# poloclub/3d-gaussian-splat-attack

Hardware: AMD Instinct MI355X
Metric: fwd+bwd views/sec @1080p, 1M Gaussians (higher is better)
Workload: dtype f32; 1 GPU; S-nyc-1M: 1000000 Gaussians (SH degree 3), 1920x1080, one view per step per GPU, render() fwd + bwd to all attribute grads, object channels off; P=1000000, width=1920, height=1080, loop=independent views, views_per_rank=1, views_per_launch_chain=1, cameras=the 8 ring cameras in turn, streams=4, parallelism=views sharded 1/GPU, dp1, independent views pipelined over 4 HIP streams per GPU

## Files before the change

3d-gaussian-splat-attack_amd/csrc/gsr_api.hip:

```cpp
#include <hip/hip_runtime.h>
#include <hip/hip_ext.h>

#include <algorithm>
#include <atomic>
#include <cfloat>
#include <cmath>
#include <cstdarg>
#include <cstdio>
#include <cstdlib>
#include <cstring>
#include <chrono>
#include <mutex>
#include <thread>
#include <new>
#include <vector>

#include "../../include/gsraster.h"
#include "gsr_kernels.hip.h"
#include "gsr_sort.hip.h"
#include "gsr_knn.hip.h"
#include "gsr_pgd.hip.h"
#include "gsr_groups.hip.h"
#include "gsr_hull.h"
#include "gsr_image.hip.h"
// ... 227 lines not shown
    const CapKey& q = g_caps[i].k;
    if (q.dev == k.dev && q.P == k.P && q.H == k.H && q.W == k.W) {
      if (erase) { g_caps[i] = g_caps.back(); g_caps.pop_back(); }
      else g_caps[i].n = n;
      return;
    }
  }
  if (!erase) {
    if (g_caps.size() >= 256) g_caps.clear();
    g_caps.push_back(CapEntry{k, n});
  }
}

struct SideStream { int dev; hipStream_t main, side; hipEvent_t fork, join; };
std::mutex g_side_mu;
std::vector<SideStream> g_sides;

bool side_stream_for(int dev, hipStream_t main, SideStream& out) {
  std::lock_guard<std::mutex> lk(g_side_mu);
  for (const SideStream& s : g_sides)
    if (s.dev == dev && s.main == main) { out = s; return true; }
  SideStream s{dev, main, nullptr, nullptr, nullptr};
  int least = 0, greatest = 0;
  if (hipDeviceGetStreamPriorityRange(&least, &greatest) != hipSuccess) { (void)hipGetLastError(); least = 0; }
  if (hipStreamCreateWithPriority(&s.side, hipStreamNonBlocking, least) != hipSuccess ||
      hipEventCreateWithFlags(&s.fork, hipEventDisableTiming) != hipSuccess ||
      hipEventCreateWithFlags(&s.join, hipEventDisableTiming) != hipSuccess) {
    (void)hipGetLastError();
    return false;
  }
  g_sides.push_back(s);
  out = s;
  return true;
}

struct PendingSlot { CountSlot slot; CapKey key; };
std::mutex g_pending_mu;
std::vector<PendingSlot> g_pending;

void pending_harvest() {
  std::lock_guard<std::mutex> lk(g_pending_mu);
  for (size_t i = 0; i < g_pending.size();) {
    PendingSlot& ps = g_pending[i];
    if (slot_landed(ps.slot)) {
      const unsigned long long n = (unsigned long long)ps.slot.host[HS_N64] | ((unsigned long long)ps.slot.host[HS_N64 + 1] << 32);
      cap_store(ps.key, n, ps.slot.host[HS_OVF] != 0u);
      slot_put(ps.slot);
      g_pending[i] = g_pending.back();
      g_pending.pop_back();
    } else {
      ++i;
    }
  }
}

struct ProfSpan { int stage; hipEvent_t a, b; };
std::mutex g_prof_mu;
uint32_t g_prof = 0;
std::vector<ProfSpan> g_spans;
std::vector<hipEvent_t> g_free_events;
float g_ms[GSR_STAGE_COUNT] = {0};
int64_t g_calls[GSR_STAGE_COUNT] = {0};

hipEvent_t get_event_locked() {
  if (!g_free_events.empty()) { hipEvent_t e = g_free_events.back(); g_free_events.pop_back(); return e; }
  hipEvent_t e;
// ... 429 lines not shown
  }
};

int FwdRun::allocate() {
  c = new (std::nothrow) GsrCtx();
  if (!c) return set_err(GSR_ERR_NOMEM, "gsr_forward: host allocation failed");
  c->dev = dev; c->st = *f.s; c->P = p.P; c->K = p.K; c->gridx = p.gridx; c->gridy = p.gridy; c->ntiles = p.ntiles;
  c->B = p.B; c->Ppad = p.Ppad; c->Pv = p.Pv; c->tpv = p.tpv;
  if (p.B > 1) c->views.assign(f.s, f.s + p.B);
  c->means3D = f.means3D; c->shs = f.shs; c->sh_objs = p.sh_objs; c->colors = f.colors_precomp; c->opac = f.opacities;
  c->scales = f.scales; c->rots = f.rotations; c->cov3d = f.cov3D_precomp;
  c->raw = f.raw; c->sh_dc = f.sh_dc;
  c->fwd_only = f.fwd_only; c->objects_out = f.out_objects != nullptr && p.sh_objs != nullptr;
  c->aux = f.out_depth != nullptr || f.out_alpha != nullptr; c->aux_depth_out = f.out_depth; c->aux_alpha_out = f.out_alpha;
  if (f.segb) { c->has_b = true; c->b = *f.segb; }
  c->lanegroup = p.lanegroup;
  c->depth_passes = p.depth_passes; c->group_sums = p.group_sums; c->scan_items = scan_items_for((uint32_t)p.Pv);
  Slab ksize, ssize;
  keep_regions(ksize, p, c);
  scratch_regions(ssize, p, w);
  c->keep_bytes = ksize.block_bytes();
  c->keep_blk = pool_alloc(dev, c->keep_bytes, st);
  scratch_blk = pool_alloc(dev, ssize.block_bytes(), st);
  if (!c->keep_blk || !scratch_blk)
    return set_err(GSR_ERR_NOMEM, "gsr_forward: workspace allocation failed (P=%d, %dx%d)", p.P, p.W, p.H);
  Slab ks(c->keep_blk, c->keep_bytes), ss(scratch_blk, ssize.block_bytes());
  keep_regions(ks, p, c);
  scratch_regions(ss, p, w);
  if (!ks.ok || !ss.ok) return set_err(GSR_ERR_STATE, "gsr_forward: a workspace region ends beyond its block");
  return GSR_OK;
}

int FwdRun::fork_color() {
  static const int side_env = [] { const char* e = getenv("GSR_SIDE_STREAM"); return e ? atoi(e) : 1; }();
  hipStream_t cs = st;
  if (side_env != 0 && !(f.s->flags & GSR_FLAG_NO_SIDE_STREAM) && side_stream_for(dev, st, side)) {
    HIP_TRY("side stream", hipEventRecord(side.fork, st));
    HIP_TRY("side stream", hipStreamWaitEvent(side.side, side.fork, 0));
    cs = side.side;
    side_used = true;
  }
  constexpr unsigned COLOR_BLOCKS = 512;
  const dim3 gridC(side_used ? std::min<unsigned>(p.nkc, COLOR_BLOCKS) : p.nkc), blkCol(PREF_BLOCK);
  if (p.B > 1) hipLaunchKernelGGL(k_pre_color_batch, gridC, blkCol, 0, cs, color_batch_args(c, w.tcnt));
  else hipLaunchKernelGGL(f.raw ? k_pre_color<true> : k_pre_color<false>, gridC, blkCol, 0, cs, color_args(c, w.tcnt));
  if (side_used) HIP_TRY("side stream", hipEventRecord(side.join, side.side));
  return GSR_OK;
}

int FwdRun::preprocess() {
  const int ntiles = p.ntiles;
  StageTimer t(GSR_STAGE_PREPROCESS, st);
  PreBlockOut bo;
  bo.bout = w.bout;
  bo.ranges = p.P >= p.tpv ? c->ranges : nullptr;
  bo.ntiles = p.tpv;
  if (!bo.ranges) {
    HIP_TRY("ranges", hipMemset2DAsync(c->ranges, sizeof(uint2), 0xFF, sizeof(uint32_t), ntiles, st));
    HIP_TRY("ranges", hipMemset2DAsync(reinterpret_cast<char*>(c->ranges) + sizeof(uint32_t), sizeof(uint2), 0, sizeof(uint32_t), ntiles, st));
  }
  if (p.B > 1) launch_pack_views(c, st);
  if (c->lanegroup) {
    PreArgs pa = color_args(c, w.tcnt);
    pa.Pfill = p.B > 1 ? p.Ppad : p.P; pa.vpack = p.B > 1 ? c->vpack : nullptr; pa.bpv = (int)p.nk1v;
    pa.scales = f.scales; pa.rots = f.rotations; pa.cov3d = f.cov3D_precomp; pa.opac = f.opacities;
    pa.colors = f.colors_precomp; pa.radii = f.radii; pa.dkey = w.dkey; pa.tcnt8 = w.tcnt8; pa.abc = c->abc;
    pa.scales_b = f.segb ? f.segb->scaling : nullptr; pa.rots_b = f.segb ? f.segb->rotation : nullptr;
    pa.opac_b = f.segb ? f.segb->opacity : nullptr;
    pa.cull = p.cull; pa.bo = bo;
// ... 447 lines not shown
  if (c->P > 0) {
    StageTimer t(GSR_STAGE_PREPROCESS, st);
    const bool skip_D = (flags & GSR_RERENDER_COLOR_GRADS_ONLY) != 0u;
    c->D_stale = c->D != nullptr && skip_D;
    const bool first_only = c->has_b && (flags & GSR_RERENDER_FIRST_SEGMENT_ONLY);
    const dim3 blkC(PREF_BLOCK);
    if (c->B > 1) {
      launch_pack_views(c, st);
      PreColorBatchArgs ca = color_batch_args(c, nullptr);
      if (first_only) ca.P = ca.Pa;
      if (skip_D) ca.D = nullptr;
      hipLaunchKernelGGL(k_pre_color_batch, dim3((unsigned)((ca.P + PREF_BLOCK - 1) / PREF_BLOCK)), blkC, 0, st, ca);
    } else {
      PreArgs pa = color_args(c, nullptr);
      if (first_only) pa.P = pa.Pa;
      if (skip_D) pa.D = nullptr;
      hipLaunchKernelGGL(c->raw ? k_pre_color<true> : k_pre_color<false>, dim3((unsigned)((pa.P + PREF_BLOCK - 1) / PREF_BLOCK)), blkC, 0, st, pa);
    }
    hipError_t e = hipGetLastError();
    if (e != hipSuccess)
      return set_err(GSR_ERR_DEVICE, "rerender colours%s: launch failed: %s", c->B > 1 ? " (batch)" : "", hipGetErrorString(e));
  }
  StageTimer t(GSR_STAGE_RENDER_FWD, st);
  return launch_render_fwd(c, out_color, out_objects, st);
}

}

static bool batch_k9_fused() {
  static const int env = [] { const char* e = getenv("GSR_BATCH_K9"); return e ? atoi(e) : 1; }();
  return env != 0;
}

struct GradOut {
  float *means3D = nullptr, *means2D = nullptr, *shs = nullptr, *sh_dc = nullptr, *sh_objs = nullptr,
        *colors_precomp = nullptr, *opacities = nullptr, *scales = nullptr, *rotations = nullptr, *cov3D = nullptr;
};

struct BwdCall {
  const float *grad_color = nullptr, *grad_objects = nullptr;
  GradOut d;
  bool accumulate = false;
  int nchunks = 1;
  gsr_chunk_fn chunk_done = nullptr;
  void* chunk_user = nullptr;
  int64_t view_stride = 0;
  void* stream = nullptr;
};

static int check_ctx_kind(const char* fn, const GsrCtx* c, bool want_raw) {
  if (!c || c->raw == want_raw) return GSR_OK;
  if (!want_raw) return set_err(GSR_ERR_STATE, "%s: context came from gsr_forward_raw; use gsr_backward_raw", fn);
  return set_err(GSR_ERR_STATE, "%s: context came from gsr_forward; use gsr_backward", fn);
}

struct BwdRun {
  GsrCtx* c;
  const BwdCall& b;
  hipStream_t st;
  double* ss_out = nullptr;
  const float *aux_gd = nullptr, *aux_ga = nullptr;
  bool aux = false;
  bool obj = false;
  bool geom = false;
  int nchunks = 1;
  bool batch_fused = false;
  bool segs_on = false;
  int bwd_npx = 4;
  uint32_t nsub = 1;
  uint32_t tag_lo = 0, tag_hi = 0;
  float4 *part = nullptr, *part_obj = nullptr;
  int finish(int code) { pool_free(c->dev, part); pool_free(c->dev, part_obj); return code; }

  int check_aux_grads() const;
  int check_pre_bwd();
  int take_partial_rows();
  int render_bwd();
  int pre_bwd();
  PreBwdArgs shared_args() const;
  void launch_batch(const PreBwdArgs& sh, int gb, int ge) const;
  void launch_views(PreBwdArgs pa, int gb, int ge) const;
  void launch_view(PreBwdArgs pa, int v, int gb, int ge) const;
};

int BwdRun::check_aux_grads() const {
  if (b.view_stride != 0)
    return set_err(GSR_ERR_INVALID, "gsr_ctx_set_aux_grads: the per-view batch backward (gsr_backward_raw_batch_views / _obj_views) "
                   "does not take depth / alpha gradients");
  if (b.nchunks > 1)
    return set_err(GSR_ERR_INVALID, "gsr_ctx_set_aux_grads: gsr_backward_raw_chunked with more than one range does not take "
                   "depth / alpha gradients");
  if (b.grad_objects != nullptr)
    return set_err(GSR_ERR_INVALID, "gsr_ctx_set_aux_grads: depth / alpha gradients and grad_objects in one backward are not supported");
  if (!geom)
    return set_err(GSR_ERR_INVALID, "gsr_ctx_set_aux_grads: depth / alpha gradients reach geometry and opacity only, and this "
                   "backward asks for no such gradient");
  if (!c->lanegroup)
    return set_err(GSR_ERR_INVALID, "gsr_ctx_set_aux_grads: a gsr_forward context with K != 16 SH coefficients does not take "
                   "depth / alpha gradients");
  if (c->st.flags & GSR_FLAG_NEEDLE_DOUBLE)
    return set_err(GSR_ERR_INVALID, "gsr_ctx_set_aux_grads: not available under GSR_FLAG_NEEDLE_DOUBLE");
  return GSR_OK;
}

int BwdRun::check_pre_bwd() {
  const float* const dsh = c->shs ? b.d.shs : nullptr;
  if (c->raw && ((dsh == nullptr) != (b.d.sh_dc == nullptr)))
    return set_err(GSR_ERR_INVALID, "gsr_backward_raw: dfeatures_dc and dfeatures_rest must both be given");
  if (c->lanegroup && c->shs && geom && !c->D)
    return set_err(GSR_ERR_STATE, "gsr_backward: the forward of this context was run without its backward state");
  if (c->lanegroup && c->shs && geom && c->D_stale)
    return set_err(GSR_ERR_STATE, "gsr_backward: geometry gradients asked of a context whose last gsr_ctx_rerender was "
                   "told GSR_RERENDER_COLOR_GRADS_ONLY");
  nchunks = std::max(1, std::min(b.nchunks, (c->P + 63) / 64));
  batch_fused = c->B > 1 && c->raw && c->lanegroup && batch_k9_fused() && b.view_stride == 0;
  if (ss_out && (!(c->lanegroup && c->raw) || b.accumulate || nchunks != 1 || (c->B > 1 && !batch_fused)))
    return set_err(GSR_ERR_INVALID, "gsr_ctx_request_sumsq: served by an overwriting gsr_backward_raw* over one range only");
  return GSR_OK;
}

int BwdRun::take_partial_rows() {
  const uint32_t N = c->nbound;
  segs_on = c->bnd != nullptr && !obj && aux_gd == nullptr;
  bwd_npx = flag_bwd_npx(c->st.flags) ? flag_bwd_npx(c->st.flags) : ((c->tpv < 4096 && !segs_on) ? 2 : 4);
  nsub = (uint32_t)(PXL / bwd_npx);
  if (N > 0) {
    part = static_cast<float4*>(pool_alloc(c->dev, sizeof(float4) * PART_F4 * (size_t)N * nsub, st));
    if (obj) part_obj = static_cast<float4*>(pool_alloc(c->dev, sizeof(float4) * 4 * (size_t)N * nsub, st));
    if (!part || (obj && !part_obj))
      return set_err(GSR_ERR_NOMEM, "gsr_backward: partial-gradient buffer (N=%u) allocation failed", N);
  }
  static std::atomic<uint64_t> tag_counter{0x243F6A8885A308D3ull};
  uint64_t z = tag_counter.fetch_add(0x9E3779B97F4A7C15ull) + 0x9E3779B97F4A7C15ull;
  z = (z ^ (z >> 30)) * 0xBF58476D1CE4E5B9ull; z = (z ^ (z >> 27)) * 0x94D049BB133111EBull; z ^= z >> 31;
  tag_lo = (uint32_t)z; tag_hi = (uint32_t)(z >> 32);
  return GSR_OK;
}

int BwdRun::render_bwd() {
  StageTimer t(GSR_STAGE_RENDER_BWD, st, true);
  RenderBwdArgs ra;
  ra.tag_lo = tag_lo; ra.tag_hi = tag_hi;
  ra.ranges = c->ranges; ra.pair_rank = c->pair_rank; ra.offg = c->offg; ra.R0 = c->G0; ra.R1 = c->G1; ra.R2 = c->G2;
  ra.sh_objs = c->sh_objs; ra.bg = c->st.bg; ra.W = c->st.image_width; ra.H = c->st.image_height;
  ra.map_mode = flag_tile_map(c->st.flags);
  ra.sched = c->sched;
  ra.wave_clock = g_wave_clock.load();
  ra.gridx = c->gridx; ra.ntiles = c->ntiles; ra.final_T = c->final_T; ra.n_contrib = c->n_contrib;
  ra.grad_color = b.grad_color; ra.grad_objects = obj ? b.grad_objects : nullptr; ra.part = part; ra.part_obj = part_obj;
  ra.grad_depth = aux_gd; ra.grad_alpha = aux_ga;
  ra.bnd = segs_on ? c->bnd : nullptr; ra.segoff = c->segoff; ra.rec_item = c->rec_item; ra.nrec = c->dv + DV_NREC;
  ra.seg_shift = c->seg_shift; ra.extra_blocks = segs_on ? c->rec_cap * nsub : 0u;
  ra.tpv = c->tpv; ra.vpack = c->vpack; ra.Ppad = c->Ppad;
  const dim3 gridT(ra.extra_blocks + (unsigned)render_grid(c->ntiles * (int)nsub)), blk(64);
  const Kern<RenderBwdArgs> k7 = pick_render_bwd(obj, bwd_npx, geom, aux);
  if (t.on) hipExtLaunchKernelGGL(k7, gridT, blk, 0, st, t.a, t.b, 0, ra);
  else hipLaunchKernelGGL(k7, gridT, blk, 0, st, ra);
  LAUNCH_CHECK("render backward");
  return GSR_OK;
}

PreBwdArgs BwdRun::shared_args() const {
  const GradOut& g = b.d;
  PreBwdArgs pa;
  pa.P = c->P; pa.g0 = 0; pa.K = c->K; pa.va = view_args(c->st);
  pa.offg = c->offg; pa.G0 = c->G0; pa.G1 = c->G1; pa.G2 = c->G2;
  pa.part = part; pa.part_obj = obj ? part_obj : nullptr;
  pa.tag_lo = tag_lo; pa.tag_hi = tag_hi; pa.nsub = nsub;
  pa.means = c->means3D; pa.scales = c->scales; pa.rots = c->rots; pa.cov3d = c->cov3d; pa.sh = c->shs;
  pa.sh_dc = c->sh_dc; pa.D = c->D; pa.abc = c->abc;
  pa.needle_double = (c->st.flags & GSR_FLAG_NEEDLE_DOUBLE) != 0u ? 1 : 0;
  pa.dmeans3D = g.means3D; pa.dmeans2D = g.means2D; pa.dsh = c->shs ? g.shs : nullptr; pa.dsh_dc = g.sh_dc;
  pa.dsh_objs = c->B > 1 ? nullptr : g.sh_objs; pa.dcolors = c->colors ? g.colors_precomp : nullptr; pa.dopac = g.opacities;
  pa.dscales = c->cov3d ? nullptr : g.scales; pa.drots = c->cov3d ? nullptr : g.rotations;
  pa.dcov3d = c->cov3d ? g.cov3D : nullptr;
  pa.accumulate = b.accumulate ? 1 : 0;
  pa.vpack = nullptr; pa.Ppad = 0; pa.Pscene = c->P; pa.vstride = 0;
  pa.sumsq = nullptr;
  return pa;
}

void BwdRun::launch_batch(const PreBwdArgs& sh, int gb, int ge) const {
  const GradOut& d = b.d;
  PreBwdBatchArgs ba;
  ba.P = ge; ba.g0 = gb; ba.B = c->B; ba.Ppad = c->Ppad; ba.Pscene = c->P; ba.vpack = c->vpack;
  ba.H = c->st.image_height; ba.W = c->st.image_width; ba.deg = c->st.sh_degree; ba.mod = c->st.scale_modifier;
  ba.offg = c->offg; ba.G0 = c->G0; ba.G1 = c->G1; ba.G2 = c->G2; ba.part = part;
  ba.tag_lo = tag_lo; ba.tag_hi = tag_hi; ba.nsub = nsub;
  ba.means = c->means3D; ba.scales = c->scales; ba.rots = c->rots; ba.D = c->D;
  ba.dmeans3D = d.means3D; ba.dmeans2D = d.means2D; ba.dsh = d.shs; ba.dsh_dc = d.sh_dc; ba.dopac = d.opacities;
  ba.dscales = d.scales; ba.drots = d.rotations; ba.sumsq = sh.sumsq;
  const dim3 gridB((unsigned)((ge - gb + 63) / 64)), blkB(64 * BATCH_K9_WAVES);
  const size_t lds = sizeof(float) * 3 * 64 * (size_t)c->B;
  hipLaunchKernelGGL(pick_pre_bwd_batch(geom, b.accumulate, aux), gridB, blkB, lds, st, ba);
}

void BwdRun::launch_views(PreBwdArgs pa, int gb, int ge) const {
  pa.vpack = c->vpack; pa.Ppad = c->Ppad; pa.Pscene = c->P; pa.vstride = (long long)b.view_stride;
  pa.accumulate = 0; pa.abc = nullptr;
  pa.g0 = gb; pa.P = ge;
  const dim3 gridV((unsigned)((ge - gb + PRE_BLOCK - 1) / PRE_BLOCK), (unsigned)c->B);
  hipLaunchKernelGGL(pick_pre_bwd(true, geom, false, false, false), gridV, dim3(PRE_BLOCK), 0, st, pa);
}

void BwdRun::launch_view(PreBwdArgs pa, int v, int gb, int ge) const {
  const GradOut& d = b.d;
  const bool acc_v = b.view_stride == 0 && (b.accumulate || v > 0);
  if (c->B > 1) {
    const size_t o = (size_t)v * (size_t)c->Ppad;
    pa.va = view_args(c->views[v]);
    pa.offg = c->offg + o; pa.G0 = c->G0 + REC * o; pa.G1 = c->G1 + REC * o; pa.G2 = c->G2 + REC * o;
    pa.D = c->D ? c->D + 9 * o : nullptr; pa.abc = c->abc ? c->abc + o : nullptr;
    pa.dmeans2D = d.means2D ? d.means2D + 3 * (size_t)v * (size_t)c->P : nullptr;
    pa.accumulate = acc_v ? 1 : 0;
  }
  pa.g0 = gb; pa.P = ge;
  const dim3 gridK9((unsigned)((ge - gb + PRE_BLOCK - 1) / PRE_BLOCK));
  if (c->lanegroup) {
    const bool ndl = pa.needle_double != 0 && pa.abc != nullptr;
    hipLaunchKernelGGL(pick_pre_bwd(c->raw, geom, acc_v, ndl, aux), gridK9, dim3(PRE_BLOCK), 0, st, pa);
  } else {
    if (geom && pa.needle_double) hipLaunchKernelGGL((k_preprocess_bwd<true, true>), gridK9, dim3(PRE_BLOCK), 0, st, pa);
    else if (geom) hipLaunchKernelGGL((k_preprocess_bwd<true>), gridK9, dim3(PRE_BLOCK), 0, st, pa);
    else hipLaunchKernelGGL((k_preprocess_bwd<false>), gridK9, dim3(PRE_BLOCK), 0, st, pa);
  }
}

int BwdRun::pre_bwd() {
  const int P = c->P, dev = c->dev;
  StageTimer t(GSR_STAGE_PREPROCESS_BWD, st);
  PreBwdArgs pa = shared_args();
  if (c->B > 1 && b.d.sh_objs) {
// ... 24 lines not shown
  if (ss_out) {
    hipLaunchKernelGGL(k_sumsq_reduce, dim3(6), dim3(256), 0, st, pa.sumsq, ss_blocks * PRE_WAVES, ss_out);
    pool_free(dev, ss_blk);
  }
  LAUNCH_CHECK("preprocess backward");
  return GSR_OK;
}

static int backward_impl(GsrCtx* c, const BwdCall& b) {
  if (!c) return set_err(GSR_ERR_STATE, "gsr_backward: null context");
  BwdRun r{c, b, static_cast<hipStream_t>(b.stream)};
  r.ss_out = c->sumsq_out;
  c->sumsq_out = nullptr;
  r.aux_gd = c->aux_gd; r.aux_ga = c->aux_ga;
  c->aux_gd = nullptr; c->aux_ga = nullptr;
  r.aux = r.aux_gd != nullptr || r.aux_ga != nullptr;
  if (!b.grad_color) return set_err(GSR_ERR_INVALID, "gsr_backward: grad_color is null");
  if (c->fwd_only)
    return set_err(GSR_ERR_STATE, "gsr_backward: the context was kept by gsr_forward_raw2_keep (re-render only, no backward state)");
  if (c->P == 0) return GSR_OK;
  const GradOut& d = b.d;
  r.obj = b.grad_objects != nullptr && c->sh_objs != nullptr;
  r.geom = d.means3D || d.means2D || d.opacities || d.scales || d.rotations || d.cov3D;
  if (r.aux) { if (const int rc = r.check_aux_grads()) return rc; }
  if (ctx_resolve_count(c) != GSR_OK) return set_err(GSR_ERR_DEVICE, "gsr_backward: reading the forward's pair count failed");
  if (c->overflow)
    return set_err(GSR_ERR_OVERFLOW, "gsr_backward: the forward emitted %llu (tile, Gaussian) pairs, more than the capacity "
                   "%u guessed from earlier views (GSR_FLAG_ASYNC_COUNT); its image was filled with NaN -- render again",
                   c->n64, c->nbound);
  if (const int rc = r.check_pre_bwd()) return rc;
  pool_retag(c->dev, c->keep_blk, r.st); pool_retag(c->dev, c->rank_blk, r.st); pool_retag(c->dev, c->seg_blk, r.st);
  int rc;
  if ((rc = r.take_partial_rows()) != GSR_OK) return r.finish(rc);
  if (c->nbound > 0 && (rc = r.render_bwd()) != GSR_OK) return r.finish(rc);
  if ((rc = r.pre_bwd()) != GSR_OK) return r.finish(rc);
  return r.finish(GSR_OK);
}

static inline size_t det_round(size_t v) { return (v + 255) & ~(size_t)255; }

struct Carve {
  char* base;
  size_t off = 0;
  explicit Carve(void* ws = nullptr) : base(static_cast<char*>(ws)) {}
  template <class T>
  T* take(size_t count) {
    T* p = base ? reinterpret_cast<T*>(base + off) : nullptr;
    off += det_round(count * sizeof(T));
    return p;
  }
};

static int check_workspace(const char* fn, const void* ws, int64_t ws_bytes, size_t need, unsigned align, const char* sizer) {
  if (ws_bytes < (int64_t)need)
    return set_err(GSR_ERR_INVALID, "%s: workspace of %lld bytes, %zu needed (%s)", fn, (long long)ws_bytes, need, sizer);
  if (((uintptr_t)ws & (uintptr_t)(align - 1)) != 0)
    return set_err(GSR_ERR_INVALID, "%s: the workspace must be %u-byte aligned", fn, align);
  return GSR_OK;
}

template <class... P>
static int check_aligned4(const char* fn, const P*... p) {
  if (((... | (uintptr_t)p) & 3) != 0) return set_err(GSR_ERR_INVALID, "%s: every tensor must be 4-byte aligned", fn);
  return GSR_OK;
}

// ... 1623 lines not shown
```

3d-gaussian-splat-attack_amd/csrc/gsr_kernels.hip.h:

```cpp
#pragma once
#include <hip/hip_runtime.h>
#include <stdint.h>

#include "gsr_math.h"
#include "gsr_sort.hip.h"

namespace gsr {

struct ViewArgs {
  const float* vm;
  const float* pm;
  const float* cam;
  int H, W;
  float tanfovx, tanfovy, mod;
  int deg;
};

__device__ __forceinline__ void load_view(View& v, const ViewArgs& a) {
  make_view(v, a.vm, a.pm, a.cam, a.H, a.W, a.tanfovx, a.tanfovy, a.mod, a.deg);
}

constexpr int MAX_BATCH = 16;
constexpr int BATCH_PAD = 16384;
struct ViewDev {
// ... 1193 lines not shown
  ViewArgs va;
  const uint32_t* offg;
  const float4* G0;
  const float4* G1;
  const float4* G2;
  const float4* part;
  const float4* part_obj;
  uint32_t tag_lo, tag_hi;
  uint32_t nsub;
  const float* means;
  const float* scales;
  const float* rots;
  const float* cov3d;
  const float* sh;
  const float* sh_dc;
  const float* D;
  const double* abc;
  float* dmeans3D;
  float* dmeans2D;
  float* dsh;
  float* dsh_dc;
  float* dsh_objs;
  float* dcolors;
  float* dopac;
  float* dscales;
  float* drots;
  float* dcov3d;
  int accumulate;
  int needle_double;
  float* sumsq;
  const ViewDev* vpack;
  int Ppad, Pscene;
  long long vstride;
};
enum { SUMSQ_XYZ = 0, SUMSQ_DC = 1, SUMSQ_REST = 2, SUMSQ_OPACITY = 3, SUMSQ_SCALING = 4, SUMSQ_ROTATION = 5, SUMSQ_W = 8 };

__global__ void __launch_bounds__(256) k_sumsq_reduce(const float* __restrict__ part, int nblocks, double* __restrict__ out) {
  __shared__ double wsum[4];
  const int k = blockIdx.x;
  double acc = 0.0;
  for (int i = threadIdx.x; i < nblocks; i += 256) acc += (double)part[(size_t)i * SUMSQ_W + k];
#pragma unroll
  for (int s = 32; s > 0; s >>= 1) acc += __shfl_xor(acc, s, 64);
  if ((threadIdx.x & 63) == 0) wsum[threadIdx.x >> 6] = acc;
  __syncthreads();
  if (threadIdx.x == 0) out[k] = (wsum[0] + wsum[1]) + (wsum[2] + wsum[3]);
}

template <bool GEOM, bool NDL = false>
__global__ void __launch_bounds__(PRE_BLOCK) k_preprocess_bwd(PreBwdArgs a) {
  const int g = a.g0 + blockIdx.x * PRE_BLOCK + threadIdx.x;
  const int K = a.K;
  if (g >= a.P) return;
  const uint32_t o0 = a.offg[g] * a.nsub, o1 = a.offg[g + 1] * a.nsub;
  if (o1 == o0) {
    if (a.dmeans3D) { a.dmeans3D[3 * g] = 0.f; a.dmeans3D[3 * g + 1] = 0.f; a.dmeans3D[3 * g + 2] = 0.f; }
    if (a.dmeans2D) { a.dmeans2D[3 * g] = 0.f; a.dmeans2D[3 * g + 1] = 0.f; a.dmeans2D[3 * g + 2] = 0.f; }
    if (a.dsh) for (int i = 0; i < 3 * K; ++i) a.dsh[(size_t)g * K * 3 + i] = 0.f;
    if (a.dsh_objs) for (int i = 0; i < NUM_OBJ; ++i) a.dsh_objs[(size_t)g * NUM_OBJ + i] = 0.f;
    if (a.dcolors) { a.dcolors[3 * g] = 0.f; a.dcolors[3 * g + 1] = 0.f; a.dcolors[3 * g + 2] = 0.f; }
    if (a.dopac) a.dopac[g] = 0.f;
    if (a.dscales) { a.dscales[3 * g] = 0.f; a.dscales[3 * g + 1] = 0.f; a.dscales[3 * g + 2] = 0.f; }
    if (a.drots) { a.drots[4 * g] = 0.f; a.drots[4 * g + 1] = 0.f; a.drots[4 * g + 2] = 0.f; a.drots[4 * g + 3] = 0.f; }
    if (a.dcov3d) for (int i = 0; i < 6; ++i) a.dcov3d[6 * g + i] = 0.f;
    return;
  }
// ... 465 lines not shown

constexpr int ROW_CHUNK = 128;
constexpr int HAND_W = 7;

template <bool RAW, bool GEOM, bool ACC = false, bool NDL = false, bool AUX = false>
__global__ void __launch_bounds__(PRE_BLOCK) k_pre_bwd(PreBwdArgs a) {
  static_assert(!AUX || (GEOM && !NDL), "aux gradients: geometry chain, no double needles");
  __shared__ float4 srow[PRE_WAVES * ROW_CHUNK * PART_F4];
  __shared__ float shand[PRE_WAVES * 64 * HAND_W];
  const int lane = threadIdx.x & 63, wave = threadIdx.x >> 6;
  const int gw0 = a.g0 + blockIdx.x * PRE_BLOCK + wave * 64;
  const int g = gw0 + lane;
  float4* wrow = &srow[wave * ROW_CHUNK * PART_F4];
  float* hand = &shand[wave * 64 * HAND_W];
  const int nw = min(64, a.P - gw0);
  if (nw <= 0) return;
  const int vw = a.vpack != nullptr ? (int)blockIdx.y : 0;
  if (a.vpack != nullptr) {
    const size_t o = (size_t)vw * (size_t)a.Ppad;
    const size_t vs = (size_t)vw * (size_t)a.vstride;
    a.offg += o; a.G0 += REC * o; a.G1 += REC * o; a.G2 += REC * o;
    if (a.D) a.D += 9 * o;
    if (a.dmeans2D) a.dmeans2D += 3 * (size_t)vw * (size_t)a.Pscene;
    if (a.dmeans3D) a.dmeans3D += vs;
    if (a.dsh) a.dsh += vs;
    if (a.dsh_dc) a.dsh_dc += vs;
    if (a.dopac) a.dopac += vs;
    if (a.dscales) a.dscales += vs;
    if (a.drots) a.drots += vs;
  }
  uint32_t o0 = 0, o1 = 0;
  if (g < a.P) { o0 = a.offg[g] * a.nsub; o1 = a.offg[g + 1] * a.nsub; }
  constexpr bool acc = ACC;
  auto put = [](float* p, float v) { if (ACC) *p += v; else *p = v; };
  float4 e0 = make_float4(0.f, 0.f, 0.f, 0.f), e1 = e0, e2 = e0;
  float p[3] = {0.f, 0.f, 0.f};
  if (o1 != o0) {
    e0 = a.G0[REC * g]; e1 = a.G1[REC * g]; e2 = a.G2[REC * g];
    p[0] = a.means[3 * g]; p[1] = a.means[3 * g + 1]; p[2] = a.means[3 * g + 2];
  }
  float dop = 0.f, dr = 0.f, dg = 0.f, db = 0.f;
  float dzv = 0.f;
  double mx = 0.0, my = 0.0, mxx = 0.0, mxy = 0.0, myy = 0.0;
  {
    const uint32_t S = a.offg[gw0] * a.nsub, E = a.offg[gw0 + nw] * a.nsub;
    const bool big = (o1 - o0) > (uint32_t)ROW_CHUNK;
    for (uint32_t c0 = S; c0 < E; c0 += (uint32_t)ROW_CHUNK) {
      const uint32_t rows = min((uint32_t)ROW_CHUNK, E - c0);
      const float4* src = a.part + (size_t)c0 * PART_F4;
      for (uint32_t i = lane; i < rows * PART_F4; i += 64) wrow[i] = src[i];
      __builtin_amdgcn_fence(__ATOMIC_RELEASE, "wavefront");
      __builtin_amdgcn_wave_barrier();
      __builtin_amdgcn_fence(__ATOMIC_ACQUIRE, "wavefront");
      if (!big) {
        const uint32_t lo = max(o0, c0), hi = min(o1, c0 + rows);
        for (uint32_t e = lo; e < hi; ++e) {
          const float4* r = &wrow[(e - c0) * PART_F4];
          const float4 p0 = r[0], p1 = r[1], p2 = r[2];
          if (__float_as_uint(p2.y) != a.tag_lo || __float_as_uint(p2.z) != a.tag_hi) continue;
          if (GEOM) { mx += (double)p0.x; my += (double)p0.y; mxx += (double)p0.z; mxy += (double)p0.w; myy += (double)p1.x; dop += p1.y; }
          dr += p1.z; dg += p1.w; db += p2.x;
          if constexpr (AUX) dzv += p2.w;
        }
      }
      __builtin_amdgcn_fence(__ATOMIC_RELEASE, "wavefront");
      __builtin_amdgcn_wave_barrier();
// ... 15 lines not shown
        if constexpr (AUX) tz += p2.w;
      }
      if constexpr (AUX) { tz = __shfl(wave_sum_to_hi(tz), 63, 64); if (lane == L) dzv = tz; }
#pragma unroll
      for (int i = 0; i < 9; ++i) t[i] = __shfl(wave_sum_to_hi(t[i]), 63, 64);
      if (GEOM) {
#pragma unroll
        for (int i = 0; i < 5; ++i) {
#pragma unroll
          for (int sft = 32; sft > 0; sft >>= 1) t2[i] += __shfl_xor(t2[i], sft, 64);
        }
      }
      if (lane == L) { mx = t2[3]; my = t2[4]; mxx = t2[0]; mxy = t2[1]; myy = t2[2]; dop = t[5]; dr = t[6]; dg = t[7]; db = t[8]; }
    }
  }
  float hdir[3] = {0.f, 0.f, 0.f}, hrgb[3] = {0.f, 0.f, 0.f};
  float ssq[6] = {0.f, 0.f, 0.f, 0.f, 0.f, 0.f};
  const bool want_ss = RAW && !ACC && a.sumsq != nullptr;
  static_assert(PRE_WAVES == 1, "more waves per workgroup: empty waves must zero their sum-of-squares slot");
  auto flush_sumsq = [&]() {
    if (!want_ss) return;
#pragma unroll
    for (int k = 0; k < 6; ++k) ssq[k] = wave_sum_to_hi(ssq[k]);
    if (lane == 63) {
      float* dst = a.sumsq + (size_t)(blockIdx.x * PRE_WAVES + wave) * SUMSQ_W;
#pragma unroll
      for (int k = 0; k < 6; ++k) dst[k] = ssq[k];
    }
  };
  if (g < a.P) {
    if (o1 == o0 && acc) {
      if (a.dmeans2D) { a.dmeans2D[3 * g] = 0.f; a.dmeans2D[3 * g + 1] = 0.f; a.dmeans2D[3 * g + 2] = 0.f; }
      if (a.dsh_objs) for (int i = 0; i < NUM_OBJ; ++i) a.dsh_objs[(size_t)g * NUM_OBJ + i] = 0.f;
    } else if (o1 == o0) {
      if (a.dmeans3D) { a.dmeans3D[3 * g] = 0.f; a.dmeans3D[3 * g + 1] = 0.f; a.dmeans3D[3 * g + 2] = 0.f; }
      if (a.dmeans2D) { a.dmeans2D[3 * g] = 0.f; a.dmeans2D[3 * g + 1] = 0.f; a.dmeans2D[3 * g + 2] = 0.f; }
      if (a.dsh_objs) for (int i = 0; i < NUM_OBJ; ++i) a.dsh_objs[(size_t)g * NUM_OBJ + i] = 0.f;
      if (a.dcolors) { a.dcolors[3 * g] = 0.f; a.dcolors[3 * g + 1] = 0.f; a.dcolors[3 * g + 2] = 0.f; }
      if (a.dopac) a.dopac[g] = 0.f;
      if (a.dscales) { a.dscales[3 * g] = 0.f; a.dscales[3 * g + 1] = 0.f; a.dscales[3 * g + 2] = 0.f; }
      if (a.drots) { a.drots[4 * g] = 0.f; a.drots[4 * g + 1] = 0.f; a.drots[4 * g + 2] = 0.f; a.drots[4 * g + 3] = 0.f; }
      if (a.dcov3d) for (int i = 0; i < 6; ++i) a.dcov3d[6 * g + i] = 0.f;
    } else {
      if (a.dsh_objs) {
        float acc_o[NUM_OBJ];
#pragma unroll
        for (int c = 0; c < NUM_OBJ; ++c) acc_o[c] = 0.f;
        if (a.part_obj) {
          for (uint32_t e = o0; e < o1; ++e) {
            const float4 tg = a.part[(size_t)e * PART_F4 + 2];
            if (__float_as_uint(tg.y) != a.tag_lo || __float_as_uint(tg.z) != a.tag_hi) continue;
#pragma unroll
            for (int q = 0; q < 4; ++q) {
              const float4 v4 = a.part_obj[(size_t)e * 4 + q];
              acc_o[4 * q] += v4.x; acc_o[4 * q + 1] += v4.y; acc_o[4 * q + 2] += v4.z; acc_o[4 * q + 3] += v4.w;
            }
          }
        }
#pragma unroll
        for (int c = 0; c < NUM_OBJ; ++c) a.dsh_objs[(size_t)g * NUM_OBJ + c] = acc_o[c];
      }
      View v;
      if (a.vpack != nullptr) {
        const ViewDev& vd = a.vpack[vw];
        make_view(v, vd.vm, vd.pm, vd.cam, a.va.H, a.va.W, vd.tanfovx, vd.tanfovy, a.va.mod, a.va.deg);
      } else {
// ... 68 lines not shown
          }
          ds[0] = (float)dsd[0]; ds[1] = (float)dsd[1]; ds[2] = (float)dsd[2];
          dq[0] = (float)dqd[0]; dq[1] = (float)dqd[1]; dq[2] = (float)dqd[2]; dq[3] = (float)dqd[3];
        } else {
          project_splat_bwd(v, p, c6, dA, dB, dC, dndcx, dndcy, dp, dc6);
        }
        if (a.dmeans3D) {
          put(&a.dmeans3D[3 * g], dp[0]); put(&a.dmeans3D[3 * g + 1], dp[1]); put(&a.dmeans3D[3 * g + 2], dp[2]);
          ssq[SUMSQ_XYZ] = dp[0] * dp[0] + dp[1] * dp[1] + dp[2] * dp[2];
        }
        if (a.cov3d) {
          if (a.dcov3d) for (int i = 0; i < 6; ++i) put(&a.dcov3d[6 * g + i], dc6[i]);
        } else if (a.dscales || a.drots) {
          if (!(NDL && needle)) {
            cov3d_bwd(sc, a.va.mod, q, dc6, ds, dq);
            if (RAW) {
              ds[0] *= sc[0]; ds[1] *= sc[1]; ds[2] *= sc[2];
              act_normalize4_bwd(q, inv_qn, dq, dq);
            }
          }
          if (a.dscales) {
            put(&a.dscales[3 * g], ds[0]); put(&a.dscales[3 * g + 1], ds[1]); put(&a.dscales[3 * g + 2], ds[2]);
            ssq[SUMSQ_SCALING] = ds[0] * ds[0] + ds[1] * ds[1] + ds[2] * ds[2];
          }
          if (a.drots) {
            put(&a.drots[4 * g], dq[0]); put(&a.drots[4 * g + 1], dq[1]); put(&a.drots[4 * g + 2], dq[2]); put(&a.drots[4 * g + 3], dq[3]);
            ssq[SUMSQ_ROTATION] = dq[0] * dq[0] + dq[1] * dq[1] + dq[2] * dq[2] + dq[3] * dq[3];
          }
        }
      }
    }
  }
  if (a.dsh == nullptr) { flush_sumsq(); return; }
  {
    float* h = hand + HAND_W * lane;
    h[0] = hdir[0]; h[1] = hdir[1]; h[2] = hdir[2]; h[3] = hrgb[0]; h[4] = hrgb[1]; h[5] = hrgb[2];
    h[6] = (o1 != o0) ? 1.f : 0.f;
  }
  __builtin_amdgcn_fence(__ATOMIC_RELEASE, "wavefront");
  __builtin_amdgcn_wave_barrier();
  __builtin_amdgcn_fence(__ATOMIC_ACQUIRE, "wavefront");
  const int q = lane & 3, grp = lane >> 2;
  const int deg = a.va.deg;
#pragma unroll 1
  for (int r0 = 0; r0 < nw; r0 += 16) {
    const int si = r0 + grp;
    if (si < nw) {
      const float* h = hand + HAND_W * si;
      const float x = h[0], y = h[1], z = h[2], g0 = h[3], g1 = h[4], g2 = h[5];
      float b[16];
#pragma unroll
      for (int k = 0; k < 16; ++k) b[k] = 0.f;
      sh_basis(deg, x, y, z, b);
      float out[12];
#pragma unroll
      for (int j = 0; j < 4; ++j) {
        const float bj = pick4(q, b[j], b[4 + j], b[8 + j], b[12 + j]);
        out[3 * j] = bj * g0; out[3 * j + 1] = bj * g1; out[3 * j + 2] = bj * g2;
      }
      if (acc) {
        if (h[6] != 0.f) {
          float cur[12];
          load_sh12<RAW>(a.dsh, a.dsh_dc, (uint32_t)(gw0 + si), q, cur);
#pragma unroll
          for (int j = 0; j < 12; ++j) out[j] += cur[j];
          store_sh12<RAW>(a.dsh, a.dsh_dc, (uint32_t)(gw0 + si), q, out);
        }
      } else {
        store_sh12<RAW>(a.dsh, a.dsh_dc, (uint32_t)(gw0 + si), q, out);
        if (want_ss) {
          const float head = out[0] * out[0] + out[1] * out[1] + out[2] * out[2];
          float rest = 0.f;
#pragma unroll
          for (int j = 3; j < 12; ++j) rest = fmaf(out[j], out[j], rest);
          ssq[SUMSQ_DC] += q == 0 ? head : 0.f;
          ssq[SUMSQ_REST] += q == 0 ? rest : rest + head;
        }
      }
    }
  }
  flush_sumsq();
}

struct ObjGradBatchArgs {
  int P, B, Ppad;
  uint32_t nsub, tag_lo, tag_hi;
  const uint32_t* offg;
  const float4* part;
  const float4* part_obj;
  float* dobj;
  long long vstride;
};
__global__ void __launch_bounds__(256) k_obj_grad_batch(ObjGradBatchArgs a) {
  const int g = (int)(blockIdx.x * 256 + threadIdx.x);
  if (g >= a.P) return;
  float tot[NUM_OBJ];
#pragma unroll
  for (int c = 0; c < NUM_OBJ; ++c) tot[c] = 0.f;
#pragma unroll 1
  for (int v = 0; v < a.B; ++v) {
    const size_t i = (size_t)v * (size_t)a.Ppad + (size_t)g;
    float s[NUM_OBJ];
#pragma unroll
    for (int c = 0; c < NUM_OBJ; ++c) s[c] = 0.f;
    if (a.part_obj) {
      const uint32_t o0 = a.offg[i] * a.nsub, o1 = a.offg[i + 1] * a.nsub;
      for (uint32_t e = o0; e < o1; ++e) {
        const float4 tg = a.part[(size_t)e * PART_F4 + 2];
        if (__float_as_uint(tg.y) != a.tag_lo || __float_as_uint(tg.z) != a.tag_hi) continue;
#pragma unroll
        for (int q = 0; q < 4; ++q) {
          const float4 v4 = a.part_obj[(size_t)e * 4 + q];
          s[4 * q] += v4.x; s[4 * q + 1] += v4.y; s[4 * q + 2] += v4.z; s[4 * q + 3] += v4.w;
        }
// ... 317 lines not shown
```

3d-gaussian-splat-attack_amd/diff_gaussian_rasterization/__init__.py:

```python
from __future__ import annotations

import contextlib
import ctypes
import weakref
import os
from typing import NamedTuple, Optional

import torch
from torch import nn

from ._signatures import CHUNK_FN as _CHUNK_FN, SIGNATURES

NUM_OBJECTS = 16
_LIB_NAME = "libgsraster.so"
_lib = None

FLAG_NO_CULL = 1
FLAG_NO_SEGMENTS = 1 << 16
FLAG_FWD_SHARED = 1 << 17
FLAG_ASYNC_COUNT = 1 << 18
FLAG_NO_SIDE_STREAM = 1 << 19
FLAG_NEEDLE_DOUBLE = 1 << 20
FLAG_OBJECTS_FOR_BACKWARD_ONLY = 1 << 21
_FLAGS = int(os.environ.get("GSR_FLAGS", "0"), 0)


def flag_fwd_split(npx: int) -> int:
    return {0: 0, 1: 1, 2: 2, 4: 3}[npx] << 4


def flag_bwd_split(npx: int) -> int:
    return {0: 0, 2: 1, 4: 2}[npx] << 8


def flag_tile_map(mode: int) -> int:
    return ((mode & 3) + 1) << 12


def set_flags(flags: int) -> None:
    global _FLAGS
    _FLAGS = int(flags)



@contextlib.contextmanager
def extra_flags(flags: int):
    global _FLAGS
    old = _FLAGS
    _FLAGS = old | int(flags)
    try:
        yield
    finally:
        _FLAGS = old


GSR_STAGES = ("preprocess", "depth_sort", "bin", "tile_sort", "render_fwd", "render_bwd", "preprocess_bwd")
# ... 1289 lines not shown
```

include/gsraster.h:

```cpp
#ifndef GSRASTER_H_
#define GSRASTER_H_

#include <stdint.h>

#ifdef __cplusplus
extern "C" {
#endif

#define GSR_VERSION 604
#define GSR_NUM_OBJECTS 16

enum {
  GSR_OK = 0,
  GSR_ERR_INVALID = 1,
  GSR_ERR_DEVICE = 2,
  GSR_ERR_NOMEM = 3,
  GSR_ERR_STATE = 4,
  GSR_ERR_OVERFLOW = 5,
  GSR_ERR_HULL = 6
};

#define GSR_FLAG_NONE 0u
#define GSR_FLAG_NO_CULL 1u
#define GSR_FLAG_FWD_SPLIT(n) ((uint32_t)((n) == 1 ? 1u : (n) == 2 ? 2u : (n) == 4 ? 3u : 0u) << 4)
#define GSR_FLAG_BWD_SPLIT(n) ((uint32_t)((n) == 2 ? 1u : (n) == 4 ? 2u : 0u) << 8)
#define GSR_FLAG_TILE_MAP(m) ((uint32_t)(((m) & 3u) + 1u) << 12)
#define GSR_FLAG_NO_SEGMENTS (1u << 16)
#define GSR_FLAG_FWD_SHARED (1u << 17)
#define GSR_FLAG_ASYNC_COUNT (1u << 18)
#define GSR_FLAG_NO_SIDE_STREAM (1u << 19)
#define GSR_FLAG_NEEDLE_DOUBLE (1u << 20)

#define GSR_FLAG_OBJECTS_FOR_BACKWARD_ONLY (1u << 21)

typedef struct GsrSettings {
  int32_t image_height;
  int32_t image_width;
  float tanfovx;
  float tanfovy;
  const float* bg;
  float scale_modifier;
  const float* viewmatrix;
  const float* projmatrix;
  int32_t sh_degree;
  const float* campos;
  int32_t prefiltered;
  int32_t debug;
  uint32_t flags;
} GsrSettings;

typedef struct GsrCtx GsrCtx;

int gsr_forward(const GsrSettings* settings, int32_t P, int32_t K, const float* means3D, const float* shs,
                const float* sh_objs, const float* colors_precomp, const float* opacities, const float* scales,
                const float* rotations, const float* cov3D_precomp, float* out_color, float* out_objects,
                int32_t* radii, GsrCtx** ctx_out, int64_t* num_rendered, void* stream);

int gsr_backward(GsrCtx* ctx, const float* grad_color, const float* grad_objects, float* dmeans3D, float* dmeans2D,
                 float* dshs, float* dsh_objs, float* dcolors_precomp, float* dopacities, float* dscales,
                 float* drotations, float* dcov3D, void* stream);

int gsr_forward_raw(const GsrSettings* settings, int32_t P, const float* xyz, const float* features_dc,
                    const float* features_rest, const float* objects_dc, const float* opacity_logit,
                    const float* log_scaling, const float* rotation_raw, float* out_color, float* out_objects,
                    int32_t* radii, GsrCtx** ctx_out, int64_t* num_rendered, void* stream);
int gsr_backward_raw(GsrCtx* ctx, const float* grad_color, const float* grad_objects, float* dxyz, float* dmeans2D,
// ... 343 lines not shown
```

Measured before the change: 1327 views/s.

## Zero unseen-Gaussian gradients in a side-stream kernel overlapping render backward

Adds a kernel that writes zero gradients for Gaussians with no tile contributions. It is launched on a low-priority side stream before the render backward and joined at the end of the backward. The preprocess-backward kernel then skips its zero-writes and the SH-gradient loop for unseen Gaussians, so that work overlaps the raster backward instead of running serially on the main stream. The risk is contention with the render backward for bandwidth and compute, plus one extra launch and event pair per view.

```diff
diff --git a/3d-gaussian-splat-attack_amd/csrc/gsr_api.hip b/3d-gaussian-splat-attack_amd/csrc/gsr_api.hip
--- a/3d-gaussian-splat-attack_amd/csrc/gsr_api.hip
+++ b/3d-gaussian-splat-attack_amd/csrc/gsr_api.hip
@@ -283,6 +283,11 @@
   g_sides.push_back(s);
   out = s;
   return true;
+}
+
+bool side_stream_wanted(uint32_t flags) {
+  static const int side_env = [] { const char* e = getenv("GSR_SIDE_STREAM"); return e ? atoi(e) : 1; }();
+  return side_env != 0 && !(flags & GSR_FLAG_NO_SIDE_STREAM);
 }
 
 struct PendingSlot { CountSlot slot; CapKey key; };
@@ -778,9 +783,8 @@
 }
 
 int FwdRun::fork_color() {
-  static const int side_env = [] { const char* e = getenv("GSR_SIDE_STREAM"); return e ? atoi(e) : 1; }();
   hipStream_t cs = st;
-  if (side_env != 0 && !(f.s->flags & GSR_FLAG_NO_SIDE_STREAM) && side_stream_for(dev, st, side)) {
+  if (side_stream_wanted(f.s->flags) && side_stream_for(dev, st, side)) {
     HIP_TRY("side stream", hipEventRecord(side.fork, st));
     HIP_TRY("side stream", hipStreamWaitEvent(side.side, side.fork, 0));
     cs = side.side;
@@ -1294,6 +1298,11 @@
   return env != 0;
 }
 
+static bool unseen_fill_enabled() {
+  static const int env = [] { const char* e = getenv("GSR_UNSEEN_FILL"); return e ? atoi(e) : 1; }();
+  return env != 0;
+}
+
 struct GradOut {
   float *means3D = nullptr, *means2D = nullptr, *shs = nullptr, *sh_dc = nullptr, *sh_objs = nullptr,
         *colors_precomp = nullptr, *opacities = nullptr, *scales = nullptr, *rotations = nullptr, *cov3D = nullptr;
@@ -1332,14 +1341,23 @@
   uint32_t nsub = 1;
   uint32_t tag_lo = 0, tag_hi = 0;
   float4 *part = nullptr, *part_obj = nullptr;
-  int finish(int code) { pool_free(c->dev, part); pool_free(c->dev, part_obj); return code; }
+  bool unseen_fill = false;
+  SideStream side{};
+  bool side_forked = false;
+  int finish(int code) {
+    if (side_forked) (void)hipStreamWaitEvent(st, side.join, 0);
+    pool_free(c->dev, part); pool_free(c->dev, part_obj);
+    return code;
+  }
 
   int check_aux_grads() const;
   int check_pre_bwd();
   int take_partial_rows();
+  int fill_unseen();
   int render_bwd();
   int pre_bwd();
   PreBwdArgs shared_args() const;
+  void all_views(PreBwdArgs& pa) const;
   void launch_batch(const PreBwdArgs& sh, int gb, int ge) const;
   void launch_views(PreBwdArgs pa, int gb, int ge) const;
   void launch_view(PreBwdArgs pa, int v, int gb, int ge) const;
@@ -1378,6 +1396,8 @@
   batch_fused = c->B > 1 && c->raw && c->lanegroup && batch_k9_fused() && b.view_stride == 0;
   if (ss_out && (!(c->lanegroup && c->raw) || b.accumulate || nchunks != 1 || (c->B > 1 && !batch_fused)))
     return set_err(GSR_ERR_INVALID, "gsr_ctx_request_sumsq: served by an overwriting gsr_backward_raw* over one range only");
+  unseen_fill = c->lanegroup && !b.accumulate && nchunks == 1 && b.chunk_done == nullptr && !batch_fused &&
+                (c->B == 1 || b.view_stride != 0) && unseen_fill_enabled() && !(c->st.flags & GSR_FLAG_K9_WRITES_ZEROS);
   return GSR_OK;
 }
 
@@ -1439,7 +1459,30 @@
   pa.accumulate = b.accumulate ? 1 : 0;
   pa.vpack = nullptr; pa.Ppad = 0; pa.Pscene = c->P; pa.vstride = 0;
   pa.sumsq = nullptr;
+  pa.skip_unseen = unseen_fill ? 1 : 0;
   return pa;
+}
+
+void BwdRun::all_views(PreBwdArgs& pa) const {
+  pa.vpack = c->vpack; pa.Ppad = c->Ppad; pa.Pscene = c->P; pa.vstride = (long long)b.view_stride;
+  pa.accumulate = 0; pa.abc = nullptr;
+}
+
+int BwdRun::fill_unseen() {
+  PreBwdArgs pa = shared_args();
+  if (c->B > 1) all_views(pa);
+  hipStream_t fs = st;
+  if (side_stream_wanted(c->st.flags) && side_stream_for(c->dev, st, side)) {
+    HIP_TRY("side stream", hipEventRecord(side.fork, st));
+    HIP_TRY("side stream", hipStreamWaitEvent(side.side, side.fork, 0));
+    fs = side.side;
+    side_forked = true;
+  }
+  const unsigned blocks = (unsigned)std::min((c->P + 64 * UZ_WAVES - 1) / (64 * UZ_WAVES), UZ_BLOCKS);
+  hipLaunchKernelGGL(c->raw ? k_unseen_zero<true> : k_unseen_zero<false>, dim3(blocks, (unsigned)c->B), dim3(64 * UZ_WAVES), 0, fs, pa);
+  if (side_forked) HIP_TRY("side stream", hipEventRecord(side.join, side.side));
+  LAUNCH_CHECK("unseen-Gaussian fill");
+  return GSR_OK;
 }
 
 void BwdRun::launch_batch(const PreBwdArgs& sh, int gb, int ge) const {
@@ -1458,8 +1501,7 @@
 }
 
 void BwdRun::launch_views(PreBwdArgs pa, int gb, int ge) const {
-  pa.vpack = c->vpack; pa.Ppad = c->Ppad; pa.Pscene = c->P; pa.vstride = (long long)b.view_stride;
-  pa.accumulate = 0; pa.abc = nullptr;
+  all_views(pa);
   pa.g0 = gb; pa.P = ge;
   const dim3 gridV((unsigned)((ge - gb + PRE_BLOCK - 1) / PRE_BLOCK), (unsigned)c->B);
   hipLaunchKernelGGL(pick_pre_bwd(true, geom, false, false, false), gridV, dim3(PRE_BLOCK), 0, st, pa);
@@ -1550,6 +1592,7 @@
   pool_retag(c->dev, c->keep_blk, r.st); pool_retag(c->dev, c->rank_blk, r.st); pool_retag(c->dev, c->seg_blk, r.st);
   int rc;
   if ((rc = r.take_partial_rows()) != GSR_OK) return r.finish(rc);
+  if (r.unseen_fill && (rc = r.fill_unseen()) != GSR_OK) return r.finish(rc);
   if (c->nbound > 0 && (rc = r.render_bwd()) != GSR_OK) return r.finish(rc);
   if ((rc = r.pre_bwd()) != GSR_OK) return r.finish(rc);
   return r.finish(GSR_OK);
diff --git a/3d-gaussian-splat-attack_amd/csrc/gsr_kernels.hip.h b/3d-gaussian-splat-attack_amd/csrc/gsr_kernels.hip.h
--- a/3d-gaussian-splat-attack_amd/csrc/gsr_kernels.hip.h
+++ b/3d-gaussian-splat-attack_amd/csrc/gsr_kernels.hip.h
@@ -1249,6 +1249,7 @@
   const ViewDev* vpack;
   int Ppad, Pscene;
   long long vstride;
+  int skip_unseen;
 };
 enum { SUMSQ_XYZ = 0, SUMSQ_DC = 1, SUMSQ_REST = 2, SUMSQ_OPACITY = 3, SUMSQ_SCALING = 4, SUMSQ_ROTATION = 5, SUMSQ_W = 8 };
 
@@ -1780,6 +1781,7 @@
   uint32_t o0 = 0, o1 = 0;
   if (g < a.P) { o0 = a.offg[g] * a.nsub; o1 = a.offg[g + 1] * a.nsub; }
   constexpr bool acc = ACC;
+  const bool skip = !ACC && a.skip_unseen != 0;
   auto put = [](float* p, float v) { if (ACC) *p += v; else *p = v; };
   float4 e0 = make_float4(0.f, 0.f, 0.f, 0.f), e1 = e0, e2 = e0;
   float p[3] = {0.f, 0.f, 0.f};
@@ -1861,6 +1863,7 @@
     if (o1 == o0 && acc) {
       if (a.dmeans2D) { a.dmeans2D[3 * g] = 0.f; a.dmeans2D[3 * g + 1] = 0.f; a.dmeans2D[3 * g + 2] = 0.f; }
       if (a.dsh_objs) for (int i = 0; i < NUM_OBJ; ++i) a.dsh_objs[(size_t)g * NUM_OBJ + i] = 0.f;
+    } else if (o1 == o0 && skip) {
     } else if (o1 == o0) {
       if (a.dmeans3D) { a.dmeans3D[3 * g] = 0.f; a.dmeans3D[3 * g + 1] = 0.f; a.dmeans3D[3 * g + 2] = 0.f; }
       if (a.dmeans2D) { a.dmeans2D[3 * g] = 0.f; a.dmeans2D[3 * g + 1] = 0.f; a.dmeans2D[3 * g + 2] = 0.f; }
@@ -1995,6 +1998,7 @@
     }
   }
   if (a.dsh == nullptr) { flush_sumsq(); return; }
+  if (skip && __ballot(o1 != o0) == 0) { flush_sumsq(); return; }
   {
     float* h = hand + HAND_W * lane;
     h[0] = hdir[0]; h[1] = hdir[1]; h[2] = hdir[2]; h[3] = hrgb[0]; h[4] = hrgb[1]; h[5] = hrgb[2];
@@ -2008,7 +2012,7 @@
 #pragma unroll 1
   for (int r0 = 0; r0 < nw; r0 += 16) {
     const int si = r0 + grp;
-    if (si < nw) {
+    if (si < nw && !(skip && hand[HAND_W * si + 6] == 0.f)) {
       const float* h = hand + HAND_W * si;
       const float x = h[0], y = h[1], z = h[2], g0 = h[3], g1 = h[4], g2 = h[5];
       float b[16];
@@ -2043,6 +2047,80 @@
     }
   }
   flush_sumsq();
+}
+
+constexpr int UZ_WAVES = 4;
+constexpr int UZ_BLOCKS = 128;
+template <bool RAW>
+__global__ void __launch_bounds__(64 * UZ_WAVES) k_unseen_zero(PreBwdArgs a) {
+  const int lane = threadIdx.x & 63, wave = threadIdx.x >> 6;
+  if (a.vpack != nullptr) {
+    const size_t vw = blockIdx.y;
+    const size_t vs = vw * (size_t)a.vstride;
+    a.offg += vw * (size_t)a.Ppad;
+    if (a.dmeans2D) a.dmeans2D += 3 * vw * (size_t)a.Pscene;
+    if (a.dmeans3D) a.dmeans3D += vs;
+    if (a.dsh) a.dsh += vs;
+    if (a.dsh_dc) a.dsh_dc += vs;
+    if (a.dopac) a.dopac += vs;
+    if (a.dscales) a.dscales += vs;
+    if (a.drots) a.drots += vs;
+  }
+  float z[4];
+  {
+    const int q = lane & 3;
+    float b[16];
+#pragma unroll
+    for (int k = 0; k < 16; ++k) b[k] = 0.f;
+    sh_basis(a.va.deg, 0.f, 0.f, 0.f, b);
+#pragma unroll
+    for (int j = 0; j < 4; ++j) z[j] = pick4(q, b[j], b[4 + j], b[8 + j], b[12 + j]) * 0.f;
+  }
+  auto lane_now = [&]() { uint32_t l = (uint32_t)lane; asm volatile("" : "+v"(l)); return l; };
+  const int nwave = (a.P - a.g0 + 63) >> 6;
+#pragma unroll 1
+  for (int wi = blockIdx.x * UZ_WAVES + wave; wi < nwave; wi += gridDim.x * UZ_WAVES) {
+    const int gw0 = a.g0 + 64 * wi;
+    bool un = false;
+    {
+      const int g = gw0 + (int)lane_now();
+      if (g < a.P) un = a.offg[g] == a.offg[g + 1];
+    }
+    const uint64_t um = __ballot(un);
+    if (um == 0) continue;
+    auto zero_rows = [&](float* arr, uint32_t W) {
+      float* p = arr + (size_t)gw0 * W;
+#pragma unroll 1
+      for (uint32_t w = lane_now(); w < 64u * W; w += 64u)
+        if ((um >> (w / W)) & 1) p[w] = 0.f;
+    };
+    if (a.dmeans3D) zero_rows(a.dmeans3D, 3);
+    if (a.dmeans2D) zero_rows(a.dmeans2D, 3);
+    if (a.dcolors) zero_rows(a.dcolors, 3);
+    if (a.dscales) zero_rows(a.dscales, 3);
+    if (a.dcov3d) zero_rows(a.dcov3d, 6);
+    if (a.dopac) zero_rows(a.dopac, 1);
+    auto zero_rows16 = [&](float* arr, uint32_t W4) {
+      float* p = arr + (size_t)gw0 * (4u * W4);
+#pragma unroll 1
+      for (uint32_t i = lane_now(); i < 64u * W4; i += 64u)
+        if ((um >> (i / W4)) & 1) *reinterpret_cast<F4u*>(p + 4u * i) = F4u{0.f, 0.f, 0.f, 0.f};
+    };
+    if (a.drots) zero_rows16(a.drots, 1);
+    static_assert(NUM_OBJ == 16, "four 16-byte stores per Gaussian");
+    if (a.dsh_objs) zero_rows16(a.dsh_objs, NUM_OBJ / 4);
+    if (a.dsh) {
+      const uint32_t l = lane_now();
+      const int q = (int)(l & 3u);
+#pragma unroll 1
+      for (uint32_t si = l >> 2; si < 64u; si += 16u) {
+        if ((um >> si) & 1) {
+          const float out[12] = {z[0], z[0], z[0], z[1], z[1], z[1], z[2], z[2], z[2], z[3], z[3], z[3]};
+          store_sh12<RAW>(a.dsh, a.dsh_dc, (uint32_t)gw0 + si, q, out);
+        }
+      }
+    }
+  }
 }
 
 struct ObjGradBatchArgs {
diff --git a/3d-gaussian-splat-attack_amd/diff_gaussian_rasterization/__init__.py b/3d-gaussian-splat-attack_amd/diff_gaussian_rasterization/__init__.py
--- a/3d-gaussian-splat-attack_amd/diff_gaussian_rasterization/__init__.py
+++ b/3d-gaussian-splat-attack_amd/diff_gaussian_rasterization/__init__.py
@@ -22,6 +22,7 @@
 FLAG_NO_SIDE_STREAM = 1 << 19
 FLAG_NEEDLE_DOUBLE = 1 << 20
 FLAG_OBJECTS_FOR_BACKWARD_ONLY = 1 << 21
+FLAG_K9_WRITES_ZEROS = 1 << 22
 _FLAGS = int(os.environ.get("GSR_FLAGS", "0"), 0)
 
 
diff --git a/include/gsraster.h b/include/gsraster.h
--- a/include/gsraster.h
+++ b/include/gsraster.h
@@ -32,6 +32,7 @@
 #define GSR_FLAG_NEEDLE_DOUBLE (1u << 20)
 
 #define GSR_FLAG_OBJECTS_FOR_BACKWARD_ONLY (1u << 21)
+#define GSR_FLAG_K9_WRITES_ZEROS (1u << 22)
 
 typedef struct GsrSettings {
   int32_t image_height;
```

Result: slower. 1291 views/s (-2.8%).
